# sephiroce/srf

Hardware: AMD Instinct MI355X
Metric: acoustic frames/sec through SRF (123-d fbank, 3-iter DR) at 1/2/4/8 MI355X (higher is better)
Workload: dtype fp32; 1 GPU; wsj_c4: SRF L=6 PH=CH=16 DIM=32 LPAD=RPAD=2 DR iter=3, train step (fwd+bwd+allreduce+Adam); utterances_per_gpu=28, frames_per_utterance=800, global_batch=28, parallelism=dp1, launch=hipgraph (fwd+CTC+bwd)

## Files before the change

include/srf_prof.h:

```cpp
#ifndef SRF_PROF_H_
#define SRF_PROF_H_

#ifdef __cplusplus
extern "C" {
#endif

int srf_route_dr_set_timing_events(void* const* starts, void* const* stops, int n);

#ifdef __cplusplus
}
#endif
#endif
```

srf_amd/_lib.py:

```python
import ctypes
import os

_HERE = os.path.dirname(os.path.abspath(__file__))
LIB_PATH = os.environ.get('SRF_LIB_PATH') or os.path.join(_HERE, 'libsrf.so')

_c_int, _c_size, _vp = ctypes.c_int, ctypes.c_size_t, ctypes.c_void_p

SDR_MAX_ITEMS = 8


class SdrRange(ctypes.Structure):
    _fields_ = [('t0', _c_int), ('t1', _c_int), ('emb', _vp), ('W', _vp), ('bias', _vp), ('WT', _vp),
                ('u', _vp), ('v0', _c_int), ('vn', _c_int), ('v', _vp), ('couplings', _vp),
                ('workspace', _vp), ('workspace_bytes', _c_size), ('g_v', _vp), ('carry', _vp),
                ('gu', _vp), ('g0', _c_int), ('gn', _c_int), ('g_emb', _vp), ('g_W', _vp), ('g_bias', _vp),
                ('accumulate', _c_int), ('u_bf16', _c_int), ('group', _c_int), ('gu_factored', _c_int)]


_ranges = ctypes.POINTER(SdrRange)

CAPSNORM_MAX_ITEMS = 8


class CapsnormRange(ctypes.Structure):
# ... 59 lines not shown
    'srf_cnnfe_saved_bytes': (_c_size, [_c_int] * 4),
    'srf_cnnfe_fwd_workspace': (_c_size, [_c_int] * 4),
    'srf_cnnfe_bwd_workspace': (_c_size, [_c_int] * 4),
    'srf_cnnfe_fwd': (_c_int, [_vp, _vp] + [_c_int] * 4 + [_vp] * 16 + [_c_int, ctypes.c_float, ctypes.c_ulonglong,
                                                                       _vp, _vp, _c_size, _vp, _c_size, _vp]),
    'srf_cnnfe_bwd': (_c_int, [_vp, _vp] + [_c_int] * 4 + [_vp] * 4 + [ctypes.c_float, ctypes.c_ulonglong]
                      + [_vp] * 15 + [_c_size, _vp]),
    'srf_cnnfe_bwd_parts': (_c_int, [_c_int, _vp, _vp] + [_c_int] * 4 + [_vp] * 4 + [ctypes.c_float, ctypes.c_ulonglong]
                            + [_vp] * 15 + [_c_size, _vp]),
    'srf_primary_caps_saved_bytes': (_c_size, [_c_int] * 4),
    'srf_primary_caps_bwd_workspace': (_c_size, [_c_int] * 5),
    'srf_primary_caps_fwd': (_c_int, [_vp, _vp] + [_c_int] * 5 + [_vp] * 8 + [_c_int, ctypes.c_float, ctypes.c_float,
                                                                           ctypes.c_ulonglong, _vp, _vp, _c_size, _vp]),
    'srf_primary_caps_bwd': (_c_int, [_vp, _vp] + [_c_int] * 5 + [_vp] * 5 + [_c_int, ctypes.c_float, ctypes.c_float,
                                                                           ctypes.c_ulonglong] + [_vp] * 12
                             + [_c_size, _vp]),
    'srf_primary_caps_fwd_ex': (_c_int, [_vp, _vp] + [_c_int] * 5 + [_vp] * 8
                                + [_c_int, ctypes.c_float, ctypes.c_float, ctypes.c_ulonglong, ctypes.c_float, _c_int,
                                   _vp, _vp, _c_size, _vp]),
    'srf_primary_caps_bwd_ex': (_c_int, [_vp, _vp] + [_c_int] * 5 + [_vp] * 5
                                + [_c_int, ctypes.c_float, ctypes.c_float, ctypes.c_ulonglong, ctypes.c_float]
                                + [_vp] * 12 + [_c_size, _vp]),
    'srf_capsnorm_bwd_workspace': (_c_size, [_c_int] * 3),
    'srf_capsnorm_fwd': (_c_int, [_vp, _c_int, _c_int, _vp, _vp, _c_int, ctypes.c_float, ctypes.c_ulonglong, _c_int,
                                  _vp, _vp, _vp]),
    'srf_capsnorm_bwd': (_c_int, [_vp, _c_int, _c_int, _vp, _vp, _c_int, ctypes.c_float, ctypes.c_ulonglong, _c_int]
                         + [_vp] * 6 + [_c_size, _vp]),
    'srf_capsnorm_fwd_range_n': (_c_int, [_cn_ranges] + [_c_int] * 5 + [ctypes.c_float, ctypes.c_ulonglong, _vp]),
    'srf_capsnorm_bwd_range_n': (_c_int, [_cn_ranges] + [_c_int] * 5 + [ctypes.c_float, ctypes.c_ulonglong, _vp]),
    'srf_capsnorm_fwd_range': (_c_int, [_vp] + [_c_int] * 5 + [_vp, _vp, _c_int, ctypes.c_float, ctypes.c_ulonglong,
                                                             _c_int, _vp, _vp, _vp]),
    'srf_capsnorm_bwd_range': (_c_int, [_vp] + [_c_int] * 5 + [_vp, _vp, _c_int, ctypes.c_float, ctypes.c_ulonglong,
                                                             _c_int, _vp, _vp, _vp, _vp, _vp]),
    'srf_capsnorm_params_workspace': (_c_size, [_c_int] * 2),
    'srf_capsnorm_bwd_params': (_c_int, [_vp, _c_int, _c_int, _vp, _vp, _vp, _c_size, _vp]),
    'srf_caps_head_fwd': (_c_int, [_vp, _c_int, _c_int, _c_int] + [_vp] * 4 + [_c_int, ctypes.c_float,
                                                                              ctypes.c_ulonglong, _c_int]
                          + [_vp] * 4),
    'srf_caps_head_fwd_ex': (_c_int, [_vp, _c_int, _c_int, _c_int] + [_vp] * 4
                             + [_c_int, ctypes.c_float, ctypes.c_ulonglong, _c_int, ctypes.c_float] + [_vp] * 4),
    'srf_caps_head_bwd': (_c_int, [_vp, _c_int, _c_int, _c_int] + [_vp] * 3 + [_c_int, ctypes.c_float,
                                                                              ctypes.c_ulonglong, _c_int]
                          + [_vp] * 9 + [_c_size, _vp]),
    'srf_ctc_workspace': (_c_size, [_c_int] * 4),
    'srf_ctc_loss': (_c_int, [_vp] * 4 + [_c_int] * 5 + [ctypes.c_float, _vp, _vp, _vp, _c_size, _vp]),
    'srf_ctc_align_workspace': (_c_size, [_c_int] * 4),
    'srf_ctc_align': (_c_int, [_vp] * 4 + [_c_int] * 5 + [_vp] * 6 + [_c_size, _vp]),
    'srf_edit_align_workspace': (_c_size, [_c_int] * 3),
    'srf_edit_align': (_c_int, [_vp, _vp, _c_int, _vp, _vp, _c_int, _c_int, _vp, _c_int] + [_vp] * 5
                       + [_c_int, _vp, _c_size, _vp]),
    'srf_word_split_workspace': (_c_size, [_c_int] * 2),
    'srf_word_split': (_c_int, [_vp, _vp, _c_int, _c_int, _vp, _c_int, _c_int] + [_vp] * 10 + [_c_size, _vp]),
    'srf_word_align_workspace': (_c_size, [_c_int] * 3),
    'srf_word_align': (_c_int, [_vp, _vp, _c_int, _vp, _vp, _c_int, _c_int, _vp, _c_int, _c_int] + [_vp] * 11
                       + [_c_size, _vp]),
    'srf_ctc_greedy_n': (_c_int, [_vp, _vp] + [_c_int] * 4 + [_vp, _vp, _vp, _vp]),
    'srf_ctc_greedy_frames_n': (_c_int, [_vp, _vp] + [_c_int] * 5 + [_vp, _vp, _vp, _vp, _vp]),
    'srf_ctc_beam_state_bytes': (_c_size, [_c_int] * 4),
    'srf_ctc_beam_reset': (_c_int, [_vp, _c_size] + [_c_int] * 4 + [ctypes.POINTER(_c_int), _vp]),
    'srf_ctc_beam_push_n': (_c_int, [_vp, _c_size] + [_c_int] * 5 + [_vp, _vp, _c_int, ctypes.POINTER(_c_int), _vp]),
    'srf_ctc_beam_best': (_c_int, [_vp, _c_size] + [_c_int] * 4 + [_vp, _vp, _vp, _vp]),
    'srf_ctc_beam_nbest': (_c_int, [_vp, _c_size] + [_c_int] * 6 + [_vp, _vp, _vp, _vp, _vp]),
    'srf_ctc_beam_lm_state_bytes': (_c_size, [_c_int] * 4),
    'srf_ctc_beam_lm_reset': (_c_int, [_vp, _c_size] + [_c_int] * 4 + [ctypes.POINTER(_c_int), _vp]),
    'srf_ctc_beam_lm_push_n': (_c_int, [_vp, _c_size] + [_c_int] * 5 + [_vp, _vp, _c_int, _vp, _vp, _c_int,
                                                                       ctypes.POINTER(_c_int), _vp]),
    'srf_ctc_beam_lm_best': (_c_int, [_vp, _c_size] + [_c_int] * 4 + [_vp, _vp, _vp, _vp, _vp]),
    'srf_ctc_beam_lm_nbest': (_c_int, [_vp, _c_size] + [_c_int] * 6 + [_vp, _vp, _vp, _vp, _vp, _vp]),
    'srf_mwer_workspace': (_c_size, [_c_int] * 5),
    'srf_mwer_loss': (_c_int, [_vp] * 6 + [_c_int] * 6 + [ctypes.c_float] + [_vp] * 5 + [_c_size, _vp]),
    'srf_stream_advance_n': (_c_int, [ctypes.POINTER(StreamBuf), _c_int, _c_int, _vp]),
    'srf_fbank_num_frames': (_c_int, [_c_int]),
    'srf_fbank_table_floats': (_c_size, []),
    'srf_fbank_tables': (_c_int, [_vp, _c_size]),
    'srf_fbank_static': (_c_int, [_vp, _c_int, _vp, _vp] + [_c_int] * 9 + [ctypes.c_float, ctypes.c_ulonglong, _vp, _vp]),
    'srf_fbank_deltas': (_c_int, [_vp, _vp] + [_c_int] * 6 + [_vp, _vp, _c_int, _vp, _c_int, _c_int, _vp]),
    'srf_fbank_stats': (_c_int, [_vp, _vp, _c_int, _c_int, _c_int, _vp, _vp]),
    'srf_adam_step': (_c_int, [_vp, _vp, _vp, _vp, _c_size, ctypes.c_float, ctypes.c_float, ctypes.c_float,
                               ctypes.c_float, _vp]),
}

_PROF_SIGNATURES = {
    'srf_route_dr_set_timing_events': (_c_int, [_vp, _vp, _c_int]),
}


class SrfError(RuntimeError):
    pass


_lib = None


def lib():
    global _lib
    if _lib is None:
        if not os.path.exists(LIB_PATH):
            raise ImportError(f'{LIB_PATH} is missing: build it with `make -C srf_amd/csrc` '
                              '(or __graft_entry__.build()); there is no fallback path')
        import torch
        h = ctypes.CDLL(LIB_PATH)
        for name, (res, args) in list(_SIGNATURES.items()) + list(_PROF_SIGNATURES.items()):
            fn = getattr(h, name)
            fn.restype = res
            fn.argtypes = args
        _lib = h
    return _lib


def exported_symbols():
    return list(_SIGNATURES)


def prof_symbols():
    return list(_PROF_SIGNATURES)


def check(rc, what):
    if rc != 0:
        msg = lib().srf_last_error().decode(errors='replace')
        raise SrfError(f'{what} failed (rc={rc}): {msg}')
```

srf_amd/csrc/cnnfe.hip:

```cpp
#include <algorithm>
#include <cmath>
#include <cstdlib>

#include "srf_common.h"
#include "srf_reduce.h"
#include "srf_rng.h"
#include "../../include/srf.h"

namespace {

constexpr int C = 64;
constexpr float kBnEps = 1e-3f;
constexpr float kBnMomentum = 0.99f;

struct Dims {
  int B, T, Fin;
  int T1, F1, T2, F2;
  int pt1, pf1, pt2, pf2;
};

inline int same_out(int n) { return (n + 1) / 2; }
inline int same_pad_before(int n) {
  const int out = same_out(n);
  const int total = std::max((out - 1) * 2 + 3 - n, 0);
  return total / 2;
}

Dims make_dims(int B, int T, int Fin) {
  Dims d;
  d.B = B; d.T = T; d.Fin = Fin;
  d.T1 = same_out(T); d.F1 = same_out(Fin);
  d.T2 = same_out(d.T1); d.F2 = same_out(d.F1);
  d.pt1 = same_pad_before(T); d.pf1 = same_pad_before(Fin);
  d.pt2 = same_pad_before(d.T1); d.pf2 = same_pad_before(d.F1);
  return d;
}

__device__ __forceinline__ int ceil_div_len(int len, int div) { return (len + div - 1) / div; }

__device__ __forceinline__ void chan_merge(float& n, float& mean, float& m2, float nb, float meanb, float m2b) {
  if (nb == 0.f) return;
  const float nn = n + nb;
  const float delta = meanb - mean;
  mean += delta * (nb / nn);
  m2 += m2b + delta * delta * (n * nb / nn);
  n = nn;
}

constexpr int kPackW2Threads = 2 * C * 64;
__device__ __forceinline__ void pack_w2_f16_body(int idx, const float* __restrict__ ka, const float* __restrict__ kb,
                                                 _Float16* __restrict__ wp2, float* __restrict__ wsc);
__device__ __forceinline__ void pack_w2t_f16_body(int idx, const float* __restrict__ ka, const float* __restrict__ kb,
                                                  _Float16* __restrict__ wq2h, float* __restrict__ wdsc);
constexpr int kPackW2tF16Threads = C * 64;

constexpr int kRows1 = 4;

struct Tile1 {
  int b, t1_0, fpad;
};

__device__ __forceinline__ Tile1 stage_rows1(const float* __restrict__ feats, const Dims& d, float* win) {
  const int tiles_per_b = (d.T1 + kRows1 - 1) / kRows1;
  Tile1 tl;
  tl.b = blockIdx.x / tiles_per_b;
  tl.t1_0 = (blockIdx.x - tl.b * tiles_per_b) * kRows1;
  tl.fpad = d.Fin + 2;
  const int nrows = 2 * kRows1 + 1;
  const int t_base = 2 * tl.t1_0 - d.pt1;
  for (int k = threadIdx.x; k < nrows * tl.fpad; k += blockDim.x) {
    const int r = k / tl.fpad, col = k - r * tl.fpad;
    const int t = t_base + r, f = col - 1;
    const bool ok = t >= 0 && t < d.T && f >= 0 && f < d.Fin;
    const float v = feats[((size_t)tl.b * d.T + min(max(t, 0), d.T - 1)) * d.Fin + min(max(f, 0), d.Fin - 1)];
    win[k] = ok ? v : 0.f;
  }
  __syncthreads();
  return tl;
}

__device__ __forceinline__ void window9_lds(const float* win, const Tile1& tl, const Dims& d, int w, int f1,
                                            float (&x)[9]) {
#pragma unroll
  for (int dt = 0; dt < 3; ++dt)
#pragma unroll
    for (int df = 0; df < 3; ++df) x[dt * 3 + df] = win[(2 * w + dt) * tl.fpad + 2 * f1 - d.pf1 + df + 1];
}

__global__ __launch_bounds__(256) void conv1_fwd_kernel(
    const float* __restrict__ feats, const int* __restrict__ inp_len, Dims d, const float* __restrict__ ka,
// ... 233 lines not shown
      const int idx = q * 64 * kC2Waves + tid;
      const int pl = idx >> 8, rem = idx & 255, n = rem >> 1, half = rem & 1;
      bv[q] = *reinterpret_cast<const h8*>(wp2 + pl * plane + ((size_t)tap * 2 * C + n) * C + 16 * kb + 8 * half);
    }
  };
  auto store_b = [&](int buf, const h8 (&bv)[kC2BLoads]) {
#pragma unroll
    for (int q = 0; q < kC2BLoads; ++q) {
      const int idx = q * 64 * kC2Waves + tid;
      const int pl = idx >> 8, rem = idx & 255, n = rem >> 1, half = rem & 1;
      *reinterpret_cast<h8*>(&Bs[buf][pl][n * kC2BStride + 8 * half]) = bv[q];
    }
  };
  auto load_a = [&](int kk, f4 (&av)[2], bool& ok) {
    const int tap = kk >> 2, kb = kk & 3;
    const int dt = tap / 3, df = tap - dt * 3;
    const int t1 = 2 * at2 - d.pt2 + dt, f1 = 2 * af2 - d.pf2 + df;
    ok = alive && t1 >= 0 && t1 < d.T1 && f1 >= 0 && f1 < d.F1 && t1 < alen1;
    const int t1c = min(max(t1, 0), d.T1 - 1), f1c = min(max(f1, 0), d.F1 - 1);
    const float* src = y1 + (((size_t)ab * d.T1 + t1c) * d.F1 + f1c) * C + 16 * kb + 8 * h;
    av[0] = *reinterpret_cast<const f4*>(src);
    av[1] = *reinterpret_cast<const f4*>(src + 4);
  };

  f16v acc[4];
#pragma unroll
  for (int nt = 0; nt < 4; ++nt) acc[nt] = f16v{};
  auto compute = [&](int kk, int buf, const f4 (&av)[2], bool aok) {
    h8 a1, a2;
    {
      const int c0 = 16 * (kk & 3) + 8 * h;
      float v[8];
#pragma unroll
      for (int q = 0; q < 8; ++q) {
        const float x = q < 4 ? av[0][q] : av[1][q - 4];
        v[q] = aok ? x * ss[0][c0 + q] + ss[1][c0 + q] : 0.f;
      }
      split2h8(v, a1, a2);
    }
#pragma unroll
    for (int nt = 0; nt < 4; ++nt) {
      const int nrow = (nt >> 1) * C + 32 * (nt & 1) + r;
      const h8 b1 = *reinterpret_cast<const h8*>(&Bs[buf][0][nrow * kC2BStride + 8 * h]);
      const h8 b2 = *reinterpret_cast<const h8*>(&Bs[buf][1][nrow * kC2BStride + 8 * h]);
      acc[nt] = mfma3h(a1, a2, b1, b2, acc[nt]);
    }
  };
  h8 bvA[kC2BLoads], bvB[kC2BLoads];
  f4 avA[2], avB[2], avC[2];
  bool okA, okB, okC;
  load_b(0, bvA);
  load_a(0, avA, okA);
  load_b(1, bvB);
  load_a(1, avB, okB);
  store_b(0, bvA);
  __syncthreads();
  for (int kk = 0; kk < 36; kk += 2) {
    {
      const f4 a0[2] = {avA[0], avA[1]};
      const bool ok0 = okA;
      if (kk + 2 < 36) {
        load_b(kk + 2, bvA);
        load_a(kk + 2, avA, okA);
      }
      compute(kk, 0, a0, ok0);
      store_b(1, bvB);
      __syncthreads();
    }
    {
      const f4 a1v[2] = {avB[0], avB[1]};
      const bool ok1 = okB;
      if (kk + 3 < 36) {
        load_b(kk + 3, bvB);
        load_a(kk + 3, avB, okB);
      }
      compute(kk + 1, 1, a1v, ok1);
      if (kk + 2 < 36) store_b(0, bvA);
      __syncthreads();
    }
  }
  (void)avC;
  (void)okC;

  const float keep_scale = 1.f / (1.f - drop_p);
  const float inv_b = stats1[4 * C + 1];
#pragma unroll
  for (int g = 0; g < 2; ++g) {
    const int c = 32 * g + r;
    const float bia = ba[c], bib = bb[c];
    const float sca = wsc[c] * inv_b, scb = wsc[C + c] * inv_b;
    float n = 0.f, mean = 0.f, m2 = 0.f;
#pragma unroll
    for (int q = 0; q < 4; ++q)
#pragma unroll
      for (int v = 0; v < 4; ++v) {
        const int p = p0 + 32 * wv + 8 * q + 4 * h + v;
        if (p >= P2) continue;
        const int t2 = (p / d.F2) % d.T2, b = p / (d.F2 * d.T2);
        const size_t o = (size_t)p * C + c;
        float a = acc[g][4 * q + v] * sca + bia, bvv = acc[2 + g][4 * q + v] * scb + bib;
        if (training && drop_p > 0.f) {
          bool ka, kb;
          srf_keep2(seed, kStreamConv1a, o, drop_p, ka, kb);
          a *= ka ? keep_scale : 0.f;
          bvv *= kb ? keep_scale : 0.f;
        }
        const bool sel = a >= bvv;
        float y = sel ? a : bvv;
        if (t2 >= ceil_div_len(inp_len[b], 4)) y = 0.f;
        y2[o] = y;
        sel2[o] = sel ? 1 : 0;
        n += 1.f;
        const float delta = y - mean;
        mean += delta / n;
        m2 += delta * (y - mean);
      }
    {
      float nb, mb, qb, x;
      xpair32(n, x, nb);
      nb = h ? x : nb;
      xpair32(mean, x, mb);
      mb = h ? x : mb;
      xpair32(m2, x, qb);
      qb = h ? x : qb;
      if (h == 0) chan_merge(n, mean, m2, nb, mb, qb);
    }
    if (h == 0) {
      red[0][wv][g * 32 + r] = n;
      red[1][wv][g * 32 + r] = mean;
      red[2][wv][g * 32 + r] = m2;
    }
  }
  __syncthreads();
  if (tid < 2 * 32) {
    const int gc = tid;
    float n = red[0][0][gc], mean = red[1][0][gc], m2 = red[2][0][gc];
#pragma unroll
    for (int w = 1; w < kC2Waves; ++w) chan_merge(n, mean, m2, red[0][w][gc], red[1][w][gc], red[2][w][gc]);
    part[((size_t)blockIdx.x * 3 + 0) * C + gc] = n;
    part[((size_t)blockIdx.x * 3 + 1) * C + gc] = mean;
    part[((size_t)blockIdx.x * 3 + 2) * C + gc] = m2;
  }
}

__global__ void bn_apply_kernel(const float* __restrict__ y, const float* __restrict__ stats,
                                const int* __restrict__ inp_len, int B, int Tk, int Fk, int div,
                                float* __restrict__ out) {
  const int n4 = B * Tk * Fk * C / 4;
  for (int q = blockIdx.x * blockDim.x + threadIdx.x; q < n4; q += gridDim.x * blockDim.x) {
    const int c4 = (q * 4) % C;
    const int p = q * 4 / C;
    const int t = (p / Fk) % Tk;
    const int b = p / (Fk * Tk);
    f4 v = {0.f, 0.f, 0.f, 0.f};
    if (t < ceil_div_len(inp_len[b], div)) {
      const f4 x = reinterpret_cast<const f4*>(y)[q];
      v = x * *reinterpret_cast<const f4*>(stats + 2 * C + c4) + *reinterpret_cast<const f4*>(stats + 3 * C + c4);
    }
    reinterpret_cast<f4*>(out)[q] = v;
  }
}


constexpr int kBnPx = 16;
__device__ __forceinline__ f4 wave_sum_px(f4 v) {
#pragma unroll
  for (int o = 16; o <= 32; o <<= 1) {
    v.x += __shfl_xor(v.x, o, 64); v.y += __shfl_xor(v.y, o, 64);
    v.z += __shfl_xor(v.z, o, 64); v.w += __shfl_xor(v.w, o, 64);
  }
  return v;
}

__global__ __launch_bounds__(256) void bn_bwd_reduce_kernel(const float* __restrict__ g, const float* __restrict__ y,
                                                            const float* __restrict__ stats,
                                                            const int* __restrict__ inp_len, int B, int Tk, int Fk,
                                                            int div, float* __restrict__ part) {
  __shared__ f4 sh[2][4][C / 4];
  const int lane = threadIdx.x & 63, q = lane & 15, pg = lane >> 4;
  const int wave = __builtin_amdgcn_readfirstlane(threadIdx.x >> 6);
  const f4 mean = reinterpret_cast<const f4*>(stats)[q], rstd = reinterpret_cast<const f4*>(stats + C)[q];
  const int P = B * Tk * Fk;
  f4 s0 = {0.f, 0.f, 0.f, 0.f}, s1 = s0;
  for (int p0 = (blockIdx.x * 4 + wave) * kBnPx; p0 < P; p0 += gridDim.x * 4 * kBnPx) {
    constexpr int U = kBnPx / 4;
    f4 dy[U], yv[U];
    float m[U];
#pragma unroll
    for (int u = 0; u < U; ++u) {
      const int pu = p0 + 4 * u + pg;
      const int p = min(pu, P - 1);
      const int t = (p / Fk) % Tk;
// ... 64 lines not shown
      const int b = p / (d.F2 * d.T2);
      m[u] = (pu < P && t < ceil_div_len(inp_len[b], 4)) ? 1.f : 0.f;
      gv[u] = reinterpret_cast<const f4*>(g_out)[(size_t)p * (C / 4) + q];
      yv[u] = reinterpret_cast<const f4*>(y2)[(size_t)p * (C / 4) + q];
      sv[u] = reinterpret_cast<const unsigned*>(sel2)[(size_t)p * (C / 4) + q];
    }
#pragma unroll
    for (int u = 0; u < U; ++u) {
      const int pu = p0 + 4 * u + pg;
      if (pu >= P) continue;
      const size_t o0 = (size_t)pu * C + 4 * q;
      f4 ga, gb;
#pragma unroll
      for (int e = 0; e < 4; ++e) {
        const float gy = bn_bwd_elem(gv[u][e], yv[u][e], m[u], mean[e], rstd[e], gam[e], sdy_n[e], sdyxh_n[e]);
        const bool sel = ((sv[u] >> (8 * e)) & 0xffu) != 0;
        float a = sel ? gy : 0.f, bb = sel ? 0.f : gy;
        if (drop_p > 0.f) {
          bool ka, kb;
          srf_keep2(seed, kStreamConv1a, o0 + e, drop_p, ka, kb);
          a *= ka ? keep_scale : 0.f;
          bb *= kb ? keep_scale : 0.f;
        }
        ga[e] = a;
        gb[e] = bb;
        gm = fmaxf(gm, fmaxf(fabsf(a), fabsf(bb)));
      }
      reinterpret_cast<f4*>(g_ab + (size_t)pu * 2 * C)[q] = ga;
      reinterpret_cast<f4*>(g_ab + (size_t)pu * 2 * C + C)[q] = gb;
      ga_s += ga;
      gb_s += gb;
    }
  }
  ga_s = wave_sum_px(ga_s);
  gb_s = wave_sum_px(gb_s);
  if (pg == 0) { sh[0][wave][q] = ga_s; sh[1][wave][q] = gb_s; }
#pragma unroll
  for (int o = 32; o >= 1; o >>= 1) gm = fmaxf(gm, __shfl_xor(gm, o, 64));
  if (lane == 0) smax[wave] = gm;
  __syncthreads();
  if (threadIdx.x < 2 * (C / 4)) {
    const int k = threadIdx.x / (C / 4), qq = threadIdx.x % (C / 4);
    const f4 v = sh[k][0][qq] + sh[k][1][qq] + sh[k][2][qq] + sh[k][3][qq];
    reinterpret_cast<f4*>(part + (size_t)blockIdx.x * 2 * C + k * C)[qq] = v;
  }
  if (threadIdx.x == 0 && gmax != nullptr) gmax[blockIdx.x] = fmaxf(fmaxf(smax[0], smax[1]), fmaxf(smax[2], smax[3]));
}

struct DgCls {
  int boff[5];
};

__device__ __forceinline__ void pack_w2t_f16_body(int idx, const float* __restrict__ ka, const float* __restrict__ kb,
                                                  _Float16* __restrict__ wq2h, float* __restrict__ wdsc) {
  const int cin = idx >> 6, l = idx & 63;
  float v[9][2], m = 0.f;
#pragma unroll
  for (int tap = 0; tap < 9; ++tap)
#pragma unroll
    for (int u = 0; u < 2; ++u) {
      const int n = 2 * l + u;
      v[tap][u] = (n < C ? ka : kb)[((size_t)tap * C + cin) * C + (n % C)];
      m = fmaxf(m, fabsf(v[tap][u]));
    }
#pragma unroll
  for (int o = 32; o >= 1; o >>= 1) m = fmaxf(m, __shfl_xor(m, o, 64));
  const int e = srf_split_exp(m);
  const float sc = srf_exp2i(e);
  const size_t plane = (size_t)9 * C * 2 * C;
#pragma unroll
  for (int tap = 0; tap < 9; ++tap) {
    _Float16 h1[2], h2[2];
#pragma unroll
    for (int u = 0; u < 2; ++u) srf_split2h(v[tap][u] * sc, h1[u], h2[u]);
    const size_t o = ((size_t)tap * C + cin) * 2 * C + 2 * l;
    wq2h[o] = h1[0];
    wq2h[o + 1] = h1[1];
    wq2h[plane + o] = h2[0];
    wq2h[plane + o + 1] = h2[1];
  }
  if (l == 0) wdsc[cin] = srf_exp2i(-e);
}

constexpr int kD2Waves = 4;
constexpr int kD2Px = 32 * kD2Waves;

__device__ __forceinline__ int gab_exp(const float* __restrict__ gmax, int n) {
  __shared__ float wmx[16];
  const int tid = threadIdx.x, nw = (blockDim.x + 63) >> 6;
  float m = 0.f;
  for (int k = tid; k < n; k += blockDim.x) m = fmaxf(m, gmax[k]);
#pragma unroll
  for (int o = 32; o >= 1; o >>= 1) m = fmaxf(m, __shfl_xor(m, o, 64));
  if ((tid & 63) == 0) wmx[tid >> 6] = m;
  __syncthreads();
  for (int k = 0; k < nw; ++k) m = fmaxf(m, wmx[k]);
  return srf_split_exp(m);
}

__global__ __launch_bounds__(64 * kD2Waves) __attribute__((amdgpu_waves_per_eu(2))) void conv2_dgrad32_kernel(
    const float* __restrict__ g_ab, const _Float16* __restrict__ wq2h, Dims d, DgCls cls, float* __restrict__ g_x1,
    const float* __restrict__ gmax, int ngmax, const float* __restrict__ wdsc) {
  constexpr int BCH = 2 * C * 2;
  __shared__ __attribute__((aligned(16))) _Float16 Bs[2][2][C * kC2BStride];
  const int tid = threadIdx.x;
  const int lane = tid & 63, wv = tid >> 6;
  const int r = lane & 31, h = lane >> 5;
  const int bid = blockIdx.x;
  const int c = (bid >= cls.boff[1]) + (bid >= cls.boff[2]) + (bid >= cls.boff[3]);
  const int qt = c >> 1, qf = c & 1;
  const int nkt = (d.T1 - qt + 1) / 2, nkf = (d.F1 - qf + 1) / 2;
  const int Pc = d.B * nkt * nkf;
  const int q0 = (bid - cls.boff[c]) * kD2Px;
  const int dt0 = (qt + d.pt2) & 1, df0 = (qf + d.pf2) & 1;
  const int ntf = (3 - df0 + 1) / 2, ntt = (3 - dt0 + 1) / 2;
  const int nkb = ntt * ntf * 8;
  const size_t plane = (size_t)9 * C * 2 * C;
  const int ea = gab_exp(gmax, ngmax);
  const float sa = srf_exp2i(ea), inv_sa = srf_exp2i(-ea);

  const int pa = q0 + 32 * wv + r;
  const bool alive = pa < Pc;
  const int pcl = min(pa, Pc - 1);
  const int akf = pcl % nkf, akt = (pcl / nkf) % nkt, ab = pcl / (nkf * nkt);
  const int at1 = qt + 2 * akt, af1 = qf + 2 * akf;
  auto tap_of = [&](int k) { return (dt0 + 2 * (k / ntf)) * 3 + df0 + 2 * (k % ntf); };

  constexpr int NBL = (BCH + 64 * kD2Waves - 1) / (64 * kD2Waves);
  auto load_b = [&](int kk, h8 (&bv)[NBL]) {
    const int tap = tap_of(kk >> 3), kb = kk & 7;
#pragma unroll
    for (int q = 0; q < NBL; ++q) {
      const int idx = min(q * 64 * kD2Waves + tid, BCH - 1);
      const int pl = idx / (2 * C), rem = idx % (2 * C), cin = rem >> 1, half = rem & 1;
      bv[q] = *reinterpret_cast<const h8*>(wq2h + pl * plane + ((size_t)tap * C + cin) * 2 * C + 16 * kb + 8 * half);
    }
  };
  auto store_b = [&](int buf, const h8 (&bv)[NBL]) {
#pragma unroll
    for (int q = 0; q < NBL; ++q) {
      const int idx = q * 64 * kD2Waves + tid;
      if (idx < BCH) {
        const int pl = idx / (2 * C), rem = idx % (2 * C), cin = rem >> 1, half = rem & 1;
        *reinterpret_cast<h8*>(&Bs[buf][pl][cin * kC2BStride + 8 * half]) = bv[q];
      }
    }
  };
  auto load_a = [&](int kk, f4 (&av)[2], bool& ok) {
    const int tap = tap_of(kk >> 3), kb = kk & 7;
    const int dt = tap / 3, df = tap - dt * 3;
    const int t2 = (at1 + d.pt2 - dt) >> 1, f2 = (af1 + d.pf2 - df) >> 1;
    ok = alive && t2 >= 0 && t2 < d.T2 && f2 >= 0 && f2 < d.F2;
    const int t2c = min(max(t2, 0), d.T2 - 1), f2c = min(max(f2, 0), d.F2 - 1);
    const float* src = g_ab + (((size_t)ab * d.T2 + t2c) * d.F2 + f2c) * 2 * C + 16 * kb + 8 * h;
    av[0] = *reinterpret_cast<const f4*>(src);
    av[1] = *reinterpret_cast<const f4*>(src + 4);
  };

  f16v acc[2];
  acc[0] = f16v{};
  acc[1] = f16v{};
  auto compute = [&](int buf, const f4 (&av)[2], bool aok) {
    h8 a1, a2;
    {
      float v[8];
#pragma unroll
      for (int q = 0; q < 8; ++q) v[q] = aok ? (q < 4 ? av[0][q] : av[1][q - 4]) : 0.f;
      split2h8(v, a1, a2, sa);
    }
#pragma unroll
    for (int nt = 0; nt < 2; ++nt) {
      const int nrow = 32 * nt + r;
      const h8 b1 = *reinterpret_cast<const h8*>(&Bs[buf][0][nrow * kC2BStride + 8 * h]);
      const h8 b2 = *reinterpret_cast<const h8*>(&Bs[buf][1][nrow * kC2BStride + 8 * h]);
      acc[nt] = mfma3h(a1, a2, b1, b2, acc[nt]);
    }
  };
  h8 bvA[NBL], bvB[NBL];
  f4 avA[2], avB[2];
  bool okA, okB;
  load_b(0, bvA);
  load_a(0, avA, okA);
  load_b(1, bvB);
  load_a(1, avB, okB);
  store_b(0, bvA);
  __syncthreads();
  for (int kk = 0; kk < nkb; kk += 2) {
    {
      const f4 a0[2] = {avA[0], avA[1]};
      const bool ok0 = okA;
      if (kk + 2 < nkb) {
        load_b(kk + 2, bvA);
        load_a(kk + 2, avA, okA);
      }
      compute(0, a0, ok0);
      store_b(1, bvB);
      __syncthreads();
    }
    {
      const f4 a1v[2] = {avB[0], avB[1]};
      const bool ok1 = okB;
      if (kk + 3 < nkb) {
        load_b(kk + 3, bvB);
        load_a(kk + 3, avB, okB);
      }
      compute(1, a1v, ok1);
      if (kk + 2 < nkb) store_b(0, bvA);
      __syncthreads();
    }
  }
  const float osc[2] = {inv_sa * wdsc[r], inv_sa * wdsc[32 + r]};
#pragma unroll
  for (int q = 0; q < 4; ++q)
#pragma unroll
    for (int v = 0; v < 4; ++v) {
      const int p = q0 + 32 * wv + 8 * q + 4 * h + v;
      if (p >= Pc) continue;
      const int kf = p % nkf, kt = (p / nkf) % nkt, b = p / (nkf * nkt);
      float* dst = g_x1 + (((size_t)b * d.T1 + qt + 2 * kt) * d.F1 + qf + 2 * kf) * C + r;
      dst[0] = acc[0][4 * q + v] * osc[0];
      dst[32] = acc[1][4 * q + v] * osc[1];
    }
}

constexpr int kWgChunk = 32;

struct WgDiv {
  FastDiv f2, t2;
};

constexpr int kTpPx = 64;
__global__ __launch_bounds__(256) void gab_split_t_kernel(const float* __restrict__ g_ab, int P2, int P2p,
                                                          _Float16* __restrict__ gsT, const float* __restrict__ gmax,
                                                          int ngmax) {
  __shared__ float tile[kTpPx][2 * C + 1];
  const int tid = threadIdx.x;
  const int p0 = blockIdx.x * kTpPx;
  const float sa = srf_exp2i(gab_exp(gmax, ngmax));
  for (int k = tid; k < kTpPx * (2 * C / 4); k += 256) {
    const int px = k / (2 * C / 4), q = k % (2 * C / 4);
    const int p = p0 + px;
    const f4 v = p < P2 ? *reinterpret_cast<const f4*>(g_ab + (size_t)p * 2 * C + 4 * q) : f4{0.f, 0.f, 0.f, 0.f};
    tile[px][4 * q] = v.x;
    tile[px][4 * q + 1] = v.y;
    tile[px][4 * q + 2] = v.z;
    tile[px][4 * q + 3] = v.w;
  }
  __syncthreads();
  const size_t plane = (size_t)2 * C * P2p;
  for (int task = tid; task < 2 * C * (kTpPx / 8); task += 256) {
    const int o = task & 7, n = task >> 3;
    float v[8];
#pragma unroll
    for (int k = 0; k < 8; ++k) v[k] = tile[8 * o + k][n];
    h8 p1, p2;
    split2h8(v, p1, p2, sa);
    _Float16* dst = gsT + (size_t)n * P2p + p0 + 8 * o;
    *reinterpret_cast<h8*>(dst) = p1;
    *reinterpret_cast<h8*>(dst + plane) = p2;
  }
}

constexpr int kW2Chunk = 32;
constexpr int kW2AStride = 96;

typedef short ws4 __attribute__((ext_vector_type(4)));

__device__ __forceinline__ ws4 lds_tr16(const _Float16* p) {
  return __builtin_amdgcn_ds_read_tr16_b64_v4i16(
      (__attribute__((address_space(3))) ws4*)(reinterpret_cast<uintptr_t>(p)));
}

__global__ __launch_bounds__(256) __attribute__((amdgpu_waves_per_eu(2))) void conv2_wgrad32_kernel(
    const float* __restrict__ y1, const float* __restrict__ stats1, const int* __restrict__ inp_len,
    const _Float16* __restrict__ gsT, int P2p, Dims d, WgDiv dv, int nsplit, int split_len, float* __restrict__ part,
    const float* __restrict__ gmax, int ngmax) {
  __shared__ __attribute__((aligned(16))) _Float16 As[2][2][kW2Chunk * kW2AStride];
  const float out_sc = stats1[4 * C + 1] * srf_exp2i(-gab_exp(gmax, ngmax));
  const int tid = threadIdx.x, lane = tid & 63, wv = tid >> 6;
  const int r = lane & 31, h = lane >> 5;
  const int xcd = blockIdx.x & 7, loc = blockIdx.x >> 3;
  const int tap = loc % 9, sp = xcd + 8 * (loc / 9);
  const int dt = tap / 3, df = tap - dt * 3;
  const int P2 = d.B * d.T2 * d.F2;
  const int pbeg = sp * split_len, pend = min(P2, pbeg + split_len);
  const int px = tid >> 3, oc = tid & 7;
  float scale[8], shift[8];
  const float bsc = stats1[4 * C];
#pragma unroll
  for (int k = 0; k < 8; ++k) {
    scale[k] = stats1[2 * C + 8 * oc + k] * bsc;
    shift[k] = stats1[3 * C + 8 * oc + k] * bsc;
  }
  f4 xv[2];
  bool xok = false;
  auto gather = [&](int pc0) {
    const int p = pc0 + px;
    const unsigned pcl = (unsigned)min(p, P2 - 1);
    const unsigned r1 = fdiv(pcl, dv.f2);
    const int f2 = (int)(pcl - r1 * d.F2);
    const unsigned bq = fdiv(r1, dv.t2);
    const int t2 = (int)(r1 - bq * d.T2), b = (int)bq;
    const int t1 = 2 * t2 - d.pt2 + dt, f1 = 2 * f2 - d.pf2 + df;
    xok = p < pend && t1 >= 0 && t1 < d.T1 && f1 >= 0 && f1 < d.F1 && t1 < ceil_div_len(inp_len[b], 2);
    const int t1c = min(max(t1, 0), d.T1 - 1), f1c = min(max(f1, 0), d.F1 - 1);
    const float* src = y1 + (((size_t)b * d.T1 + t1c) * d.F1 + f1c) * C + 8 * oc;
// ... 419 lines not shown

int srf_cnnfe_out_dims(int T, int feat_dim, int* T2, int* F2) {
  SRF_REQUIRE(T > 0 && feat_dim > 0 && T2 && F2, "bad arguments");
  Dims d = make_dims(1, T, feat_dim);
  *T2 = d.T2;
  *F2 = d.F2;
  return SRF_OK;
}

size_t srf_cnnfe_saved_bytes(int B, int T, int feat_dim, int nfilt) {
  (void)nfilt;
  return saved_layout(make_dims(B, T, feat_dim), nullptr).bytes;
}

size_t srf_cnnfe_fwd_workspace(int B, int T, int feat_dim, int nfilt) {
  (void)nfilt;
  return fwd_ws_layout(make_dims(B, T, feat_dim), nullptr).bytes;
}

int srf_cnnfe_fwd(const float* feats, const int* inp_len, int B, int T, int feat_dim, int nfilt,
                  const float* k0a, const float* b0a, const float* k0b, const float* b0b, const float* gamma0,
                  const float* beta0, const float* k1a, const float* b1a, const float* k1b, const float* b1b,
                  const float* gamma1, const float* beta1, float* mmean0, float* mvar0, float* mmean1, float* mvar1,
                  int training, float drop_p, unsigned long long seed, float* out, void* saved, size_t saved_bytes,
                  void* workspace, size_t workspace_bytes, void* stream) {
  int rc = check_dims(B, T, feat_dim, nfilt);
  if (rc) return rc;
  SRF_REQUIRE(feats && inp_len && k0a && b0a && k0b && b0b && gamma0 && beta0 && k1a && b1a && k1b && b1b &&
                  gamma1 && beta1 && mmean0 && mvar0 && mmean1 && mvar1 && out && saved && workspace,
              "null pointer argument");
  SRF_REQUIRE(drop_p >= 0.f && drop_p < 1.f, "dropout rate %f out of [0,1)", drop_p);
  const Dims d = make_dims(B, T, feat_dim);
  FwdSaved sv = saved_layout(d, saved);
  FwdWs w = fwd_ws_layout(d, workspace);
  if (saved_bytes < sv.bytes || workspace_bytes < w.bytes) {
    srf::set_error("CNN-FE buffers too small (saved %zu < %zu or workspace %zu < %zu)", saved_bytes, sv.bytes,
                   workspace_bytes, w.bytes);
    return SRF_EWORKSPACE;
  }
  hipStream_t st = static_cast<hipStream_t>(stream);
  const size_t P2 = (size_t)d.B * d.T2 * d.F2;
  const int nb2 = (int)((P2 + 63) / 64);
  int nparts2 = nb2;
  const int npack = (kPackW2Threads + 64 * kRows1 - 1) / (64 * kRows1);
  hipLaunchKernelGGL(conv1_fwd_kernel, dim3(conv1_blocks(d) + npack), dim3(64 * kRows1), conv1_lds(d), st, feats,
                     inp_len, d, k0a, b0a, k0b, b0b, training, drop_p, seed, srf::seed_source(), sv.y1, sv.sel1,
                     w.part1, conv1_blocks(d), k1a, k1b, w.wp2, w.wsc, w.ymax);
  SRF_LAUNCH_CHECK("conv1_fwd");
  if ((rc = bn_finalize(w.part1, conv1_blocks(d), w.merged, gamma0, beta0, mmean0, mvar0, training, sv.stats1, st,
                        w.ymax, conv1_blocks(d))))
    return rc;
  SRF_LAUNCH_CHECK("bn_finalize(1)");
  {
    const int nb32 = (int)((P2 + kC2Px - 1) / kC2Px);
    hipLaunchKernelGGL(conv2_fwd32_kernel, dim3(nb32), dim3(64 * kC2Waves), 0, st, sv.y1, sv.stats1, inp_len, d,
                       w.wp2, w.wsc, b1a, b1b, training, drop_p, seed, srf::seed_source(), sv.y2, sv.sel2,
                       w.part2);
    SRF_LAUNCH_CHECK("conv2_fwd32");
    nparts2 = nb32;
  }
  if ((rc = bn_finalize(w.part2, nparts2, w.merged, gamma1, beta1, mmean1, mvar1, training, sv.stats2, st)))
    return rc;
  SRF_LAUNCH_CHECK("bn_finalize(2)");
  hipLaunchKernelGGL(bn_apply_kernel, dim3(1024), dim3(256), 0, st, sv.y2, sv.stats2, inp_len, d.B, d.T2, d.F2, 4,
                     out);
  SRF_LAUNCH_CHECK("bn_apply");
  return SRF_OK;
}

}

namespace {
struct BwdWs2 {
  float *bnpart, *bnsum2, *bnsum1, *g_ab, *biaspart, *g_x1, *wpart, *c1part, *c1sum, *scratch;
  _Float16* wq2h;
  _Float16* gsT;
  float* gmax;
  float* wdsc;
  int P2p;
  size_t bytes;
};

constexpr int kBnBlocks = 1024;
constexpr int kWgrad32SplitsMax = 128;
constexpr int kWgrad32Splits = 56;
inline bool wgrad_by_rows(const Dims& d) { return SRF_CONV2_WGRAD_ROWS && d.F2 <= 32; }

BwdWs2 bwd_ws_layout(const Dims& d, void* base) {
  const size_t P1 = (size_t)d.B * d.T1 * d.F1, P2 = (size_t)d.B * d.T2 * d.F2;
  Bump bp;
  const size_t obp = bp.take((size_t)kBnBlocks * 2 * C * 4), os2 = bp.take(2 * C * 4), os1 = bp.take(2 * C * 4),
               oab = bp.take(P2 * 2 * C * 4), obias = bp.take((size_t)kBnBlocks * 2 * C * 4),
               ogx = bp.take(P1 * C * 4), owq = bp.take((size_t)2 * 9 * C * 2 * C * 2),
               owp = bp.take((size_t)std::max(kWgrad32SplitsMax, kWrRanges) * 9 * C * 2 * C * 4),
               oc1 = bp.take((size_t)conv1_blocks(d) * 20 * C * 4), oc1s = bp.take(20 * C * 4),
               oscr = bp.take(srf::colsum_scratch_floats(std::max(conv1_blocks(d), kBnBlocks), 20 * C) * 4);
  const int P2p = (int)((P2 + kTpPx - 1) / kTpPx * kTpPx);
  const size_t ogs = bp.take(wgrad_by_rows(d) ? 0 : (size_t)2 * 2 * C * P2p * 2);
  const size_t ogm = bp.take((size_t)kBnBlocks * 4), ods = bp.take((size_t)C * 4);
  char* b = static_cast<char*>(base);
  BwdWs2 w;
  w.bnpart = (float*)(b + obp);
  w.bnsum2 = (float*)(b + os2);
  w.bnsum1 = (float*)(b + os1);
  w.g_ab = (float*)(b + oab);
  w.biaspart = (float*)(b + obias);
  w.g_x1 = (float*)(b + ogx);
  w.wq2h = (_Float16*)(b + owq);
  w.wpart = (float*)(b + owp);
  w.c1part = (float*)(b + oc1);
  w.c1sum = (float*)(b + oc1s);
  w.scratch = (float*)(b + oscr);
  w.gsT = (_Float16*)(b + ogs);
  w.gmax = (float*)(b + ogm);
  w.wdsc = (float*)(b + ods);
  w.P2p = P2p;
  w.bytes = bp.off;
  return w;
}

}

extern "C" {

size_t srf_cnnfe_bwd_workspace(int B, int T, int feat_dim, int nfilt) {
  (void)nfilt;
  return bwd_ws_layout(make_dims(B, T, feat_dim), nullptr).bytes;
}

int srf_cnnfe_bwd(const float* feats, const int* inp_len, int B, int T, int feat_dim, int nfilt, const float* gamma0,
                  const float* k1a, const float* k1b, const float* gamma1, float drop_p, unsigned long long seed,
                  const void* saved, const float* g_out, float* g_k0a, float* g_b0a, float* g_k0b, float* g_b0b,
                  float* g_gamma0, float* g_beta0, float* g_k1a, float* g_b1a, float* g_k1b, float* g_b1b,
                  float* g_gamma1, float* g_beta1, void* workspace, size_t workspace_bytes, void* stream) {
  return srf_cnnfe_bwd_parts(SRF_CNNFE_BWD_ALL, feats, inp_len, B, T, feat_dim, nfilt, gamma0, k1a, k1b, gamma1, drop_p,
                             seed, saved, g_out, g_k0a, g_b0a, g_k0b, g_b0b, g_gamma0, g_beta0, g_k1a, g_b1a, g_k1b,
                             g_b1b, g_gamma1, g_beta1, workspace, workspace_bytes, stream);
}

int srf_cnnfe_bwd_parts(int parts, const float* feats, const int* inp_len, int B, int T, int feat_dim, int nfilt,
                        const float* gamma0, const float* k1a, const float* k1b, const float* gamma1, float drop_p,
                        unsigned long long seed, const void* saved, const float* g_out, float* g_k0a, float* g_b0a,
                        float* g_k0b, float* g_b0b, float* g_gamma0, float* g_beta0, float* g_k1a, float* g_b1a,
                        float* g_k1b, float* g_b1b, float* g_gamma1, float* g_beta1, void* workspace,
                        size_t workspace_bytes, void* stream) {
  SRF_REQUIRE(parts > 0 && (parts & ~SRF_CNNFE_BWD_ALL) == 0, "CNN-FE backward: bad parts mask %d", parts);
  int rc = check_dims(B, T, feat_dim, nfilt);
  if (rc) return rc;
  SRF_REQUIRE(feats && inp_len && gamma0 && k1a && k1b && gamma1 && saved && g_out && g_k0a && g_b0a && g_k0b &&
                  g_b0b && g_gamma0 && g_beta0 && g_k1a && g_b1a && g_k1b && g_b1b && g_gamma1 && g_beta1 &&
                  workspace,
              "null pointer argument");
  SRF_REQUIRE(((uintptr_t)g_out & 15) == 0 && ((uintptr_t)saved & 255) == 0 && ((uintptr_t)workspace & 255) == 0,
              "CNN-FE backward: g_out must be 16-byte and saved / workspace 256-byte aligned");
  const Dims d = make_dims(B, T, feat_dim);
  FwdSaved sv = saved_layout(d, const_cast<void*>(saved));
  BwdWs2 w = bwd_ws_layout(d, workspace);
  if (workspace_bytes < w.bytes) {
    srf::set_error("CNN-FE backward workspace too small: %zu < %zu", workspace_bytes, w.bytes);
    return SRF_EWORKSPACE;
  }
  hipStream_t st = static_cast<hipStream_t>(stream);
  const int P2 = d.B * d.T2 * d.F2;
  if (parts & SRF_CNNFE_BWD_PREP) {
    hipLaunchKernelGGL(bn_bwd_reduce_kernel, dim3(kBnBlocks), dim3(256), 0, st, g_out, sv.y2, sv.stats2, inp_len,
                       d.B, d.T2, d.F2, 4, w.bnpart);
    SRF_LAUNCH_CHECK("bn_bwd_reduce(2)");
    if ((rc = srf::colsum(w.bnpart, kBnBlocks, 2 * C, w.bnsum2, w.scratch, st,
                          srf::ColSplit{{g_beta1, g_gamma1, nullptr, nullptr}, {C, C, 0, 0}})))
      return rc;
    const int npack = (kPackW2tF16Threads + 255) / 256;
    hipLaunchKernelGGL(conv2_bwd_prep_kernel, dim3(kBnBlocks + npack), dim3(256), 0, st, g_out, sv.y2, sv.sel2,
                       sv.stats2, gamma1, w.bnsum2, inp_len, d, drop_p, seed, srf::seed_source(), w.g_ab,
                       w.biaspart, kBnBlocks, k1a, k1b, w.wq2h, w.wdsc, w.gmax);
    SRF_LAUNCH_CHECK("conv2_bwd_prep");
    if ((rc = srf::colsum(w.biaspart, kBnBlocks, 2 * C, nullptr, w.scratch, st,
                          srf::ColSplit{{g_b1a, g_b1b, nullptr, nullptr}, {C, C, 0, 0}})))
      return rc;
  }
  if (parts & SRF_CNNFE_BWD_DATA) {
    DgCls cls{};
    for (int c = 0; c < 4; ++c) {
      const int qt = c >> 1, qf = c & 1;
      const int Pc = d.B * ((d.T1 - qt + 1) / 2) * ((d.F1 - qf + 1) / 2);
      cls.boff[c + 1] = cls.boff[c] + (Pc + kD2Px - 1) / kD2Px;
    }
    hipLaunchKernelGGL(conv2_dgrad32_kernel, dim3(cls.boff[4]), dim3(64 * kD2Waves), 0, st, w.g_ab,
                       (const _Float16*)w.wq2h, d, cls, w.g_x1, (const float*)w.gmax, kBnBlocks,
                       (const float*)w.wdsc);
    SRF_LAUNCH_CHECK("conv2_dgrad32");
  }
  const WgDiv dv{make_fastdiv(d.F2), make_fastdiv(d.T2)};
  const int nsplit = kWgrad32Splits;
  if ((parts & SRF_CNNFE_BWD_WGRAD) && wgrad_by_rows(d)) {
    const int rows_per = (d.B * d.T2 + kWrRanges - 1) / kWrRanges;
    hipLaunchKernelGGL(conv2_wgrad_rows_kernel, dim3(2 * kWrRanges), dim3(256), 0, st, sv.y1, sv.stats1, inp_len,
                       (const float*)w.g_ab, d, rows_per, w.wpart, (const float*)w.gmax, kBnBlocks);
    SRF_LAUNCH_CHECK("conv2_wgrad_rows");
    hipLaunchKernelGGL(conv2_wgrad_reduce_rows_kernel, dim3(9 * C * 2 * C / 128), dim3(256), 0, st, w.wpart, g_k1a,
                       g_k1b);
    SRF_LAUNCH_CHECK("conv2_wgrad_reduce_rows");
  } else if (parts & SRF_CNNFE_BWD_WGRAD) {
    static_assert(kW2Chunk == kWgChunk, "wgrad splits are whole chunks");
    const int split_len = ((P2 + nsplit - 1) / nsplit + kWgChunk - 1) / kWgChunk * kWgChunk;
    hipLaunchKernelGGL(gab_split_t_kernel, dim3(w.P2p / kTpPx), dim3(256), 0, st, w.g_ab, P2, w.P2p, w.gsT,
                       (const float*)w.gmax, kBnBlocks);
    SRF_LAUNCH_CHECK("gab_split_t");
    hipLaunchKernelGGL(conv2_wgrad32_kernel, dim3(9 * nsplit), dim3(256), 0, st, sv.y1, sv.stats1, inp_len,
                       (const _Float16*)w.gsT, w.P2p, d, dv, nsplit, split_len, w.wpart, (const float*)w.gmax,
                       kBnBlocks);
    SRF_LAUNCH_CHECK("conv2_wgrad32");
    hipLaunchKernelGGL(conv2_wgrad_reduce_kernel, dim3((9 * C * 2 * C + 255) / 256), dim3(256), 0, st, w.wpart,
                       nsplit, g_k1a, g_k1b);
    SRF_LAUNCH_CHECK("conv2_wgrad_reduce");
  }
  if (!(parts & SRF_CNNFE_BWD_DATA)) return SRF_OK;
  hipLaunchKernelGGL(bn_bwd_reduce_kernel, dim3(kBnBlocks), dim3(256), 0, st, w.g_x1, sv.y1, sv.stats1, inp_len, d.B,
                     d.T1, d.F1, 2, w.bnpart);
  SRF_LAUNCH_CHECK("bn_bwd_reduce(1)");
  if ((rc = srf::colsum(w.bnpart, kBnBlocks, 2 * C, w.bnsum1, w.scratch, st, srf::ColSplit{{g_beta0, g_gamma0, nullptr, nullptr}, {C, C, 0, 0}})))
    return rc;
  hipLaunchKernelGGL(conv1_bwd_kernel, dim3(conv1_blocks(d)), dim3(64 * kRows1), conv1_lds(d), st, feats, inp_len, d, w.g_x1, sv.y1,
                     sv.sel1, sv.stats1, gamma0, w.bnsum1, drop_p, seed, srf::seed_source(), w.c1part);
  SRF_LAUNCH_CHECK("conv1_bwd");
  if ((rc = srf::colsum(w.c1part, conv1_blocks(d), 20 * C, nullptr, w.scratch, st,
                        srf::ColSplit{{g_k0a, g_k0b, g_b0a, g_b0b, nullptr, nullptr}, {9 * C, 9 * C, C, C, 0, 0}})))
    return rc;
  return SRF_OK;
}

}
```

Before: 3.199 million frames/s.

## Use persistent LDS-resident weight conv2 dgrad kernel sized to CU count

Replaces the per-class conv2 data-gradient kernel with a persistent kernel launched with one workgroup per CU. Each workgroup stages all relevant tap weights for a parity class into dynamic LDS with a swizzle, then loops over 32-pixel tiles while prefetching the next tile's activations. The goal is to stop reloading weights from global memory per block and to spread work evenly across CUs. It also replaces per-element pixel index decoding in the forward epilogue with wave ballots. The cost is a large LDS footprint (low occupancy), a sync per class, and a hipFuncSetAttribute call on every launch.

```diff
diff --git a/include/srf_prof.h b/include/srf_prof.h
--- a/include/srf_prof.h
+++ b/include/srf_prof.h
@@ -7,6 +7,8 @@
 
 int srf_route_dr_set_timing_events(void* const* starts, void* const* stops, int n);
 
+int srf_cnnfe_set_dgrad_workgroups(int n);
+
 #ifdef __cplusplus
 }
 #endif
diff --git a/srf_amd/_lib.py b/srf_amd/_lib.py
--- a/srf_amd/_lib.py
+++ b/srf_amd/_lib.py
@@ -165,6 +165,7 @@
 
 _PROF_SIGNATURES = {
     'srf_route_dr_set_timing_events': (_c_int, [_vp, _vp, _c_int]),
+    'srf_cnnfe_set_dgrad_workgroups': (_c_int, [_c_int]),
 }
 
 
diff --git a/srf_amd/csrc/cnnfe.hip b/srf_amd/csrc/cnnfe.hip
--- a/srf_amd/csrc/cnnfe.hip
+++ b/srf_amd/csrc/cnnfe.hip
@@ -6,6 +6,7 @@
 #include "srf_reduce.h"
 #include "srf_rng.h"
 #include "../../include/srf.h"
+#include "../../include/srf_prof.h"
 
 namespace {
 
@@ -405,6 +406,8 @@
   (void)avC;
   (void)okC;
 
+  const unsigned dead = (unsigned)__ballot(!alive) >> (4 * h);
+  const unsigned hid = (unsigned)__ballot(at2 >= ceil_div_len(inp_len[ab], 4)) >> (4 * h);
   const float keep_scale = 1.f / (1.f - drop_p);
   const float inv_b = stats1[4 * C + 1];
 #pragma unroll
@@ -418,8 +421,7 @@
 #pragma unroll
       for (int v = 0; v < 4; ++v) {
         const int p = p0 + 32 * wv + 8 * q + 4 * h + v;
-        if (p >= P2) continue;
-        const int t2 = (p / d.F2) % d.T2, b = p / (d.F2 * d.T2);
+        if ((dead >> (8 * q + v)) & 1u) continue;
         const size_t o = (size_t)p * C + c;
         float a = acc[g][4 * q + v] * sca + bia, bvv = acc[2 + g][4 * q + v] * scb + bib;
         if (training && drop_p > 0.f) {
@@ -430,7 +432,7 @@
         }
         const bool sel = a >= bvv;
         float y = sel ? a : bvv;
-        if (t2 >= ceil_div_len(inp_len[b], 4)) y = 0.f;
+        if ((hid >> (8 * q + v)) & 1u) y = 0.f;
         y2[o] = y;
         sel2[o] = sel ? 1 : 0;
         n += 1.f;
@@ -661,9 +663,6 @@
   if (l == 0) wdsc[cin] = srf_exp2i(-e);
 }
 
-constexpr int kD2Waves = 4;
-constexpr int kD2Px = 32 * kD2Waves;
-
 __device__ __forceinline__ int gab_exp(const float* __restrict__ gmax, int n) {
   __shared__ float wmx[16];
   const int tid = threadIdx.x, nw = (blockDim.x + 63) >> 6;
@@ -676,6 +675,29 @@
   for (int k = 0; k < nw; ++k) m = fmaxf(m, wmx[k]);
   return srf_split_exp(m);
 }
+
+#ifndef SRF_CONV2_DGRAD_LDSW
+#define SRF_CONV2_DGRAD_LDSW 1
+#endif
+
+__device__ __forceinline__ void dgrad_store(const f16v (&acc)[2], int opix, const float (&osc)[2],
+                                            float* __restrict__ g_x1) {
+  const int r = threadIdx.x & 31, h = (threadIdx.x >> 5) & 1;
+#pragma unroll
+  for (int q = 0; q < 4; ++q)
+#pragma unroll
+    for (int v = 0; v < 4; ++v) {
+      const int px = __shfl(opix, 8 * q + 4 * h + v, 64);
+      if (px < 0) continue;
+      float* dst = g_x1 + (size_t)px * C + r;
+      dst[0] = acc[0][4 * q + v] * osc[0];
+      dst[32] = acc[1][4 * q + v] * osc[1];
+    }
+}
+
+#if !SRF_CONV2_DGRAD_LDSW
+constexpr int kD2Waves = 4;
+constexpr int kD2Px = 32 * kD2Waves;
 
 __global__ __launch_bounds__(64 * kD2Waves) __attribute__((amdgpu_waves_per_eu(2))) void conv2_dgrad32_kernel(
     const float* __restrict__ g_ab, const _Float16* __restrict__ wq2h, Dims d, DgCls cls, float* __restrict__ g_x1,
@@ -789,18 +811,135 @@
     }
   }
   const float osc[2] = {inv_sa * wdsc[r], inv_sa * wdsc[32 + r]};
-#pragma unroll
-  for (int q = 0; q < 4; ++q)
-#pragma unroll
-    for (int v = 0; v < 4; ++v) {
-      const int p = q0 + 32 * wv + 8 * q + 4 * h + v;
-      if (p >= Pc) continue;
-      const int kf = p % nkf, kt = (p / nkf) % nkt, b = p / (nkf * nkt);
-      float* dst = g_x1 + (((size_t)b * d.T1 + qt + 2 * kt) * d.F1 + qf + 2 * kf) * C + r;
-      dst[0] = acc[0][4 * q + v] * osc[0];
-      dst[32] = acc[1][4 * q + v] * osc[1];
-    }
-}
+  dgrad_store(acc, alive ? (ab * d.T1 + at1) * d.F1 + af1 : -1, osc, g_x1);
+}
+
+#else
+constexpr int kDlWaves = 8;
+constexpr int kDlTapHalves = 2 * C * 2 * C;
+constexpr size_t kDlLds = (size_t)4 * kDlTapHalves * sizeof(_Float16);
+
+__global__ __launch_bounds__(64 * kDlWaves) void conv2_dgrad_ldsw_kernel(
+    const float* __restrict__ g_ab, const _Float16* __restrict__ wq2h, Dims d, float* __restrict__ g_x1,
+    const float* __restrict__ gmax, int ngmax, const float* __restrict__ wdsc) {
+  extern __shared__ __attribute__((aligned(16))) _Float16 Wl[];
+  const int tid = threadIdx.x;
+  const int lane = tid & 63, wv = __builtin_amdgcn_readfirstlane(tid >> 6);
+  const int r = lane & 31, h = lane >> 5;
+  const size_t plane = (size_t)9 * C * 2 * C;
+  const int ea = gab_exp(gmax, ngmax);
+  const float sa = srf_exp2i(ea), inv_sa = srf_exp2i(-ea);
+  const float osc[2] = {inv_sa * wdsc[r], inv_sa * wdsc[32 + r]};
+  const _Float16* wrow = Wl + r * 2 * C;
+  const int swz = r & 15;
+
+  for (int c = 0; c < 4; ++c) {
+    const int qt = c >> 1, qf = c & 1;
+    const int nkt = (d.T1 - qt + 1) / 2, nkf = (d.F1 - qf + 1) / 2;
+    const int Pc = d.B * nkt * nkf;
+    const int ntile = (Pc + 31) / 32;
+    const int tlo = (int)((long long)ntile * blockIdx.x / gridDim.x);
+    const int thi = (int)((long long)ntile * (blockIdx.x + 1) / gridDim.x);
+    if (tlo == thi) continue;
+    const int dt0 = (qt + d.pt2) & 1, df0 = (qf + d.pf2) & 1;
+    const int ntf = (3 - df0 + 1) / 2, ntt = (3 - dt0 + 1) / 2;
+    const int ntap = ntt * ntf;
+    auto tap_of = [&](int k) {
+      const int kt = ntf == 2 ? k >> 1 : k;
+      return (dt0 + 2 * kt) * 3 + df0 + 2 * (k - kt * ntf);
+    };
+
+    __syncthreads();
+    for (int ti = 0; ti < ntap; ++ti) {
+      const int tap = tap_of(ti);
+      h8 wvv[4];
+#pragma unroll
+      for (int q = 0; q < 4; ++q) {
+        const int idx = q * 64 * kDlWaves + tid;
+        const int pl = idx >> 10, cin = (idx >> 4) & 63, ch = idx & 15;
+        wvv[q] = *reinterpret_cast<const h8*>(wq2h + pl * plane + ((size_t)tap * C + cin) * 2 * C + 8 * ch);
+      }
+#pragma unroll
+      for (int q = 0; q < 4; ++q) {
+        const int idx = q * 64 * kDlWaves + tid;
+        const int pl = idx >> 10, cin = (idx >> 4) & 63, ch = idx & 15;
+        *reinterpret_cast<h8*>(Wl + ti * kDlTapHalves + (pl * C + cin) * 2 * C + 8 * (ch ^ (cin & 15))) = wvv[q];
+      }
+    }
+    __syncthreads();
+
+    int ab, at1, af1, opix;
+    bool alive;
+    auto decode = [&](int tile) {
+      const int pa = 32 * tile + r;
+      alive = pa < Pc;
+      const int pcl = min(pa, Pc - 1);
+      const int akf = pcl % nkf, akt = (pcl / nkf) % nkt;
+      ab = pcl / (nkf * nkt);
+      at1 = qt + 2 * akt;
+      af1 = qf + 2 * akf;
+    };
+    f4 avN[16];
+    bool okN;
+    auto issue = [&](int ti) {
+      const int tap = tap_of(ti);
+      const int dt = tap / 3, df = tap - dt * 3;
+      const int t2 = (at1 + d.pt2 - dt) >> 1, f2 = (af1 + d.pf2 - df) >> 1;
+      okN = alive && t2 >= 0 && t2 < d.T2 && f2 >= 0 && f2 < d.F2;
+      const int t2c = min(max(t2, 0), d.T2 - 1), f2c = min(max(f2, 0), d.F2 - 1);
+      const float* src = g_ab + (((size_t)ab * d.T2 + t2c) * d.F2 + f2c) * 2 * C + 8 * h;
+#pragma unroll
+      for (int kb = 0; kb < 8; ++kb) {
+        avN[2 * kb] = *reinterpret_cast<const f4*>(src + 16 * kb);
+        avN[2 * kb + 1] = *reinterpret_cast<const f4*>(src + 16 * kb + 4);
+      }
+    };
+
+    int tile = tlo + wv;
+    if (tile < thi) {
+      decode(tile);
+      issue(0);
+    }
+    for (; tile < thi; tile += kDlWaves) {
+      opix = alive ? (ab * d.T1 + at1) * d.F1 + af1 : -1;
+      f16v acc[2];
+      acc[0] = f16v{};
+      acc[1] = f16v{};
+      for (int ti = 0; ti < ntap; ++ti) {
+        f4 av[16];
+#pragma unroll
+        for (int k = 0; k < 16; ++k) av[k] = avN[k];
+        const bool ok = okN;
+        if (ti + 1 < ntap) {
+          issue(ti + 1);
+        } else if (tile + kDlWaves < thi) {
+          decode(tile + kDlWaves);
+          issue(0);
+        }
+        const _Float16* wt = wrow + ti * kDlTapHalves;
+#pragma unroll
+        for (int kb = 0; kb < 8; ++kb) {
+          h8 a1, a2;
+          {
+            float v[8];
+#pragma unroll
+            for (int q = 0; q < 8; ++q) v[q] = ok ? (q < 4 ? av[2 * kb][q] : av[2 * kb + 1][q - 4]) : 0.f;
+            split2h8(v, a1, a2, sa);
+          }
+          const int co = 8 * ((2 * kb + h) ^ swz);
+#pragma unroll
+          for (int nt = 0; nt < 2; ++nt) {
+            const h8 b1 = *reinterpret_cast<const h8*>(wt + (32 * nt) * 2 * C + co);
+            const h8 b2 = *reinterpret_cast<const h8*>(wt + (C + 32 * nt) * 2 * C + co);
+            acc[nt] = mfma3h(a1, a2, b1, b2, acc[nt]);
+          }
+        }
+      }
+      dgrad_store(acc, opix, osc, g_x1);
+    }
+  }
+}
+#endif
 
 constexpr int kWgChunk = 32;
 
@@ -1386,6 +1525,7 @@
 };
 
 constexpr int kBnBlocks = 1024;
+int g_dgrad_workgroups = 0;
 constexpr int kWgrad32SplitsMax = 128;
 constexpr int kWgrad32Splits = 56;
 inline bool wgrad_by_rows(const Dims& d) { return SRF_CONV2_WGRAD_ROWS && d.F2 <= 32; }
@@ -1427,6 +1567,12 @@
 
 extern "C" {
 
+int srf_cnnfe_set_dgrad_workgroups(int n) {
+  SRF_REQUIRE(n >= 0 && n <= 65535, "CNN-FE data gradient: bad workgroup count %d", n);
+  g_dgrad_workgroups = n;
+  return SRF_OK;
+}
+
 size_t srf_cnnfe_bwd_workspace(int B, int T, int feat_dim, int nfilt) {
   (void)nfilt;
   return bwd_ws_layout(make_dims(B, T, feat_dim), nullptr).bytes;
@@ -1482,6 +1628,21 @@
                           srf::ColSplit{{g_b1a, g_b1b, nullptr, nullptr}, {C, C, 0, 0}})))
       return rc;
   }
+#if SRF_CONV2_DGRAD_LDSW
+  if (parts & SRF_CNNFE_BWD_DATA) {
+    int grid = g_dgrad_workgroups;
+    if (grid <= 0) {
+      int dev = 0;
+      SRF_HIP_TRY(hipGetDevice(&dev));
+      SRF_HIP_TRY(hipDeviceGetAttribute(&grid, hipDeviceAttributeMultiprocessorCount, dev));
+    }
+    SRF_HIP_TRY(hipFuncSetAttribute((const void*)conv2_dgrad_ldsw_kernel, hipFuncAttributeMaxDynamicSharedMemorySize,
+                                    (int)kDlLds));
+    hipLaunchKernelGGL(conv2_dgrad_ldsw_kernel, dim3(grid), dim3(64 * kDlWaves), kDlLds, st, w.g_ab,
+                       (const _Float16*)w.wq2h, d, w.g_x1, (const float*)w.gmax, kBnBlocks, (const float*)w.wdsc);
+    SRF_LAUNCH_CHECK("conv2_dgrad_ldsw");
+  }
+#else
   if (parts & SRF_CNNFE_BWD_DATA) {
     DgCls cls{};
     for (int c = 0; c < 4; ++c) {
@@ -1494,6 +1655,7 @@
                        (const float*)w.wdsc);
     SRF_LAUNCH_CHECK("conv2_dgrad32");
   }
+#endif
   const WgDiv dv{make_fastdiv(d.F2), make_fastdiv(d.T2)};
   const int nsplit = kWgrad32Splits;
   if ((parts & SRF_CNNFE_BWD_WGRAD) && wgrad_by_rows(d)) {
```

After: 3.207 million frames/s (median of 6 runs). Within noise of the previous version (+0.3%).
